# qurator-spk/sbb_textline_detection

Measured on AMD Instinct MI355X. Metric: segmented patches/sec (448x448x3) per GPU + per-pixel label-map match vs ref, higher is better.
Workload: dtype f16x3; 1 GPU; BASELINE configs[1] x 32: 32 pages of 3500x2500 (70 tiles of 448x448 each, margin 0.1) per GPU per step, textline model, 2 classes; workload_id=page, dedupe=False, max_batch=320, lanes=2, owned_regions=1, exchange=none

## Files before the change

sbb_textline_detection_amd/csrc/api.hip:

```cpp
#include <stdarg.h>
#include <stdio.h>
#include <stdlib.h>
#include <string.h>

#include <algorithm>
#include <cmath>
#include <new>
#include <stdexcept>
#include <string>
#include <utility>
#include <vector>

#include "../../include/sbbseg.h"
#include <dlfcn.h>

#include <mutex>

#include "internal.h"
#include "region.h"

using namespace sbbseg;

namespace {

// ... 208 lines not shown
    void* comm = nullptr;
    int comm_rank = 0, comm_world = 1;
    void* d_deskew = nullptr; size_t deskew_cap = 0;
    uint8_t *d_run_page = nullptr, *d_run_mask = nullptr, *d_run_a = nullptr, *d_run_b = nullptr;
    size_t run_page_cap = 0, run_mask_cap = 0, run_a_cap = 0, run_b_cap = 0;
    int *d_cc_parent = nullptr, *d_cc_count = nullptr; size_t cc_parent_cap = 0, cc_count_cap = 0;
    bool force_host_contours = false;
    int host_contour_calls = 0;
    int* d_cc_list = nullptr;
    int* d_cc_aux = nullptr; size_t cc_aux_cap = 0;
    unsigned long long* d_cc_small = nullptr;
    bool profiling = false;
    int conv_variant = 0;
    bool ph8 = false;
    int fg_min_ksteps = 9;
    int fg_pointwise_min_ksteps = 4;
    bool ranged_walk = false;
    bool block_pq = true;
    bool unfuse_blocks = false;
    bool unfuse_stem_pool = false;
    bool no_dec_halo = false;
    bool no_expand_reduce = false;
    bool no_c3er = false;
    bool plain_gather = false;
    int contig_max_k = 0;
    int fused_heads = 0;
    int num_cus = 256;
    std::vector<PendingEvent> pending;
    std::vector<hipEvent_t> free_events;
    int owned_mode = 1;
    int region_levels = 0;
    int region_op[kRegionMaxLevels] = {0};
    uint32_t* d_rtab[2][kRegionMaxLevels] = {{nullptr}, {nullptr}};
    size_t rtab_cap[2][kRegionMaxLevels] = {{0}, {0}};
    RegionRun rr;
    double last_exec_frac = 1.0;
    std::vector<std::pair<void*, size_t>> user_bufs;
};

namespace {

int dmalloc(sbbseg_ctx* c, void** p, size_t bytes)
{
    HIPCHK(hipMalloc(p, bytes));
    c->device_bytes += bytes;
    return 0;
// ... 193 lines not shown
                    HIPCHK(launch_stem_pool_x3(sp, c->num_cus, c->stream));
                } else
                    HIPCHK(launch_stem(sp, c->precision, c->num_cus, c->stream));
            } else if (co.d_d64_wfrag && !(c->conv_variant & 3)) {
                const Tensor& st = c->tensors[co.d.src[0].tensor];
                Direct64Params dp;
                dp.src = st.buf; dp.n = n; dp.H = st.H; dp.W = st.W; dp.wfrag = co.d_d64_wfrag;
                dp.scale = co.d_scale; dp.shift = co.d_shift; dp.relu = co.d.relu; dp.out = c->tensors[co.d.out_tensor].data();
                dp.wmul = co.wmul_cls[0];
                HIPCHK(launch_direct64(dp, c->precision, c->num_cus, c->stream));
            } else if (co.fused_reduce >= 0 && !c->no_expand_reduce && !(c->conv_variant & 3)) {
                const ConvOp& ro = c->ops[co.fused_reduce].conv;
                if (co.fused_conv3 >= 0 && !c->no_c3er) {
                    const ConvOp& k3 = c->ops[co.fused_conv3].conv;
                    const Tensor& ta = c->tensors[k3.d.src[0].tensor];
                    C3ERParams cp;
                    cp.a = ta.buf; cp.x = c->tensors[co.d.residual_tensor].buf;
                    cp.y = c->tensors[co.d.out_tensor].buf; cp.a2 = c->tensors[ro.d.out_tensor].buf;
                    cp.n = n; cp.H = ta.H; cp.W = ta.W; cp.C = co.d.src[0].channels; cp.x3 = c->precision == kF16X3;
                    cp.w2frag = co.d_c3_w2; cp.w3frag = co.d_er_w3; cp.w1frag = co.d_er_w1;
                    cp.s2 = k3.d_scale; cp.h2 = k3.d_shift; cp.s3 = co.d_scale; cp.h3 = co.d_shift; cp.s1 = ro.d_scale; cp.h1 = ro.d_shift;
                    cp.wmul2 = k3.wmul_cls[0]; cp.wmul3 = co.wmul_cls[0]; cp.wmul1 = ro.wmul_cls[0];
                    cp.k0 = co.d_c3_k0;
                    HIPCHK(launch_conv3_expand_reduce(cp, c->num_cus, c->stream));
                    return 0;
                }
                ExpRedParams ep;
                ep.b = c->tensors[co.d.src[0].tensor].buf; ep.x = c->tensors[co.d.residual_tensor].buf;
                ep.y = c->tensors[co.d.out_tensor].buf; ep.a2 = c->tensors[ro.d.out_tensor].buf;
                ep.M = n * co.Ho * co.Wo; ep.C = co.d.src[0].channels; ep.x3 = c->precision == kF16X3;
                ep.w3frag = co.d_er_w3; ep.w1frag = co.d_er_w1;
                ep.s3 = co.d_scale; ep.h3 = co.d_shift; ep.s1 = ro.d_scale; ep.h1 = ro.d_shift;
                ep.wmul3 = co.wmul_cls[0]; ep.wmul1 = ro.wmul_cls[0];
                ep.dbg = 0;
#ifdef SBBSEG_PROBES
                { static const int er_dbg = getenv("SBBSEG_ER_DBG") ? atoi(getenv("SBBSEG_ER_DBG")) : 0; ep.dbg = er_dbg; }
#endif
                HIPCHK(launch_expand_reduce_x3(ep, c->num_cus, c->stream));
            } else if (runs_dec_halo(c, co)) {
                const Tensor& s0 = c->tensors[co.d.src[0].tensor];
                DecHaloParams hp;
                hp.src0 = s0.buf; hp.skip = c->tensors[co.d.src[1].tensor].buf; hp.PH = s0.H; hp.PW = s0.W; hp.n = n;
                hp.wfrag = co.d_halo_wfrag; hp.taps = co.d_halo_taps; hp.scale = co.d_scale; hp.shift = co.d_shift;
                for (int q = 0; q < 4; ++q) hp.wmul[q] = co.wmul_cls[q];
                hp.relu = co.d.relu; hp.out = c->tensors[co.d.out_tensor].data();
                if (rlv >= 0) { hp.ttab = c->rr.tab[rlv]; hp.n_tab = c->rr.total[rlv]; }
                if (c->precision == kF16X3) HIPCHK(launch_dec_halo_x3(hp, c->num_cus, c->stream));
                else HIPCHK(launch_dec_halo_f16(hp, c->num_cus, c->stream));
            } else {
                int ks = 0;
                if (c->ksplit_now && n == 1 && c->precision != kF32 && p.fast_gather && conv_tile_bc(p.cout) == 128 && !p.raw_out && !p.head_classes &&
                    p.out && p.cout % 8 == 0 &&
                    ((p.n_cls == 1 && p.osy == 1 && p.osx == 1 && p.ooy == 0 && p.oox == 0 && p.TH == p.Ho && p.TW == p.Wo) ||
                     (p.n_cls == 4 && p.osy == 2 && p.osx == 2 && p.TH == 2 * p.Ho && p.TW == 2 * p.Wo))) {
                    const long tiles = (long)p.n_cls * ((p.M + 127) / 128) * ((p.cout + 127) / 128);
                    while (ks < 4 && (tiles << (ks + 1)) <= 512 && p.total_ksteps % (2 << ks) == 0 && (p.total_ksteps >> (ks + 1)) >= 4) ++ks;
                }
// ... 289 lines not shown
        const int words = (c->num_cus + 31) / 32, half = c->num_cus / 2;
        std::vector<uint32_t> lo(words, 0u), hi(words, 0u);
        for (int i = 0; i < c->num_cus; ++i) (i < half ? lo : hi)[i / 32] |= 1u << (i % 32);
        hipError_t e0 = hipExtStreamCreateWithCUMask(&c->half_stream[0], (uint32_t)words, lo.data());
        hipError_t e1 = e0 == hipSuccess ? hipExtStreamCreateWithCUMask(&c->half_stream[1], (uint32_t)words, hi.data()) : e0;
        if (e1 == hipSuccess) e1 = hipEventCreateWithFlags(&c->ev_half[0], hipEventDisableTiming);
        if (e1 == hipSuccess) e1 = hipEventCreateWithFlags(&c->ev_half[1], hipEventDisableTiming);
        if (e1 == hipSuccess) {
            c->cu_split = true;
            c->half_cus[0] = half; c->half_cus[1] = c->num_cus - half;
        } else {
            (void)hipGetLastError();
            for (int k = 0; k < 2; ++k) {
                if (c->half_stream[k]) (void)hipStreamDestroy(c->half_stream[k]);
                if (c->ev_half[k]) (void)hipEventDestroy(c->ev_half[k]);
                c->half_stream[k] = nullptr; c->ev_half[k] = nullptr;
            }
        }
    }
    if (const char* v = getenv("SBBSEG_STAGGER_MIN_TILES")) c->stagger_min_tiles = atoi(v);
    if (const char* v = getenv("SBBSEG_DEDUPE")) c->dedupe = v[0] != '0';
    if (const char* v = getenv("SBBSEG_KSPLIT")) c->ksplit = v[0] != '0';
    if (const char* v = getenv("SBBSEG_OWNED_REGIONS")) c->owned_mode = v[0] == '0' ? 0 : (v[0] == '2' ? 2 : 1);
    if (const char* v = getenv("SBBSEG_GRID_CUS")) { const int n = atoi(v); if (n >= 8 && n <= c->num_cus) c->num_cus = n & ~7; }
    *out = c;
    return 0;
    API_END
}

int sbbseg_destroy(sbbseg_ctx* c)
{
    API_BEGIN
    if (!c) return 0;
    (void)hipSetDevice(c->device);
    if (c->stream) (void)hipStreamSynchronize(c->stream);
    if (c->lane_stream) (void)hipStreamSynchronize(c->lane_stream);
    for (int k = 0; k < 2; ++k)
        if (c->half_stream[k]) (void)hipStreamSynchronize(c->half_stream[k]);
    for (auto& t : c->tensors) {
        (void)hipFree(t.lane_buf[0]);
        (void)hipFree(t.lane_buf[1]);
    }
    std::vector<Op*> all_ops;
    for (auto& op : c->ops) {
        all_ops.push_back(&op);
        for (auto& part : op.parts) all_ops.push_back(&part);
// ... 2535 lines not shown
```

sbb_textline_detection_amd/csrc/conv3_expand_reduce.hip:

```cpp
#include "internal.h"

namespace sbbseg {

namespace {

typedef __attribute__((ext_vector_type(8))) _Float16 h8_t;
typedef __attribute__((ext_vector_type(4))) _Float16 h4_t;
typedef __attribute__((ext_vector_type(2))) _Float16 h2_t;
typedef __attribute__((ext_vector_type(4))) float f4_t;
typedef __attribute__((ext_vector_type(4))) unsigned u4_t;
typedef __attribute__((ext_vector_type(2))) unsigned u2_t;
#define LDS_AS __attribute__((address_space(3)))

template <int N> struct IC { static constexpr int value = N; };
template <int B, int E, class F> __device__ __attribute__((always_inline)) inline void static_for(F&& f)
{
    if constexpr (B < E) {
        f(IC<B>{});
        static_for<B + 1, E>(f);
    }
}

__device__ inline f4_t mma(h8_t a, h8_t b, f4_t c) { return __builtin_amdgcn_mfma_f32_16x16x32_f16(a, b, c, 0, 0, 0); }

// ... 41 lines not shown
__device__ __attribute__((always_inline)) inline void glds16_hidden(const void* gsrc, uint32_t lds_dst)
{
    uint32_t keep;
    asm volatile("s_mov_b32 %0, m0\n\ts_mov_b32 m0, %2\n\ts_nop 0\n\tglobal_load_lds_dwordx4 %1, off\n\ts_mov_b32 m0, %0"
                 : "=&s"(keep) : "v"(gsrc), "s"(lds_dst) : "memory");
}
__device__ inline u4_t make_rsrc(const void* base, uint32_t bytes)
{
    u4_t r;
    const uint64_t b = (uint64_t)(uintptr_t)base;
    r[0] = __builtin_amdgcn_readfirstlane((uint32_t)b);
    r[1] = __builtin_amdgcn_readfirstlane((uint32_t)(b >> 32) & 0xffffu);
    r[2] = __builtin_amdgcn_readfirstlane(bytes);
    r[3] = 0x00020000u;
    return r;
}

constexpr int kHaloPx = 100;
constexpr int kHaloInstr = 25;
constexpr int kPieceBytes = kHaloInstr * 1024;

}

template <int C, bool X3>
__global__ __launch_bounds__(512, 2) void conv3_expand_reduce(const C3ERParams p)
{
    static_assert(C == 128, "stage 3 only (LDS: the split mode's halo + b + y chunk fill it at C = 128)");
    constexpr int EB = X3 ? 4 : 2;
    constexpr int KCH = X3 ? 32 : 64;
    constexpr int KS0 = 9 * C / KCH;
    constexpr int KS1 = C / KCH;
    constexpr int G2S = 256 / KCH;
    constexpr int NCH = C / 64;
    constexpr int MI2 = C / 128;
    constexpr int LG2 = 2 * MI2;
    constexpr int PB = C * EB, PY = 4 * C * EB, PA = C * EB;
    constexpr int NP = PB / 256;
    constexpr int YROW = 256 * EB;
    constexpr int SLB = PB / 16, SLY = YROW / 16;
    constexpr int kHaloBytes = NP * kPieceBytes, kBBytes = 64 * PB, kYBytes = 64 * YROW;
    constexpr int PER = KS1 + G2S;
    constexpr int STEPS = KS0 + NCH * PER;
    constexpr int kEpi1 = X3 ? 16 : 8, kEpi2 = X3 ? 8 : 4;
    constexpr int kDma = 4 * NP;
    static_assert(STEPS % 2 == 0 && KS0 % 2 == 0, "the weight ring alternates two register sets");
    extern __shared__ __attribute__((aligned(16))) char smem[];
    char* const lds_a = smem;
    char* const lds_b = smem + kHaloBytes;
    char* const lds_y = lds_b + kBBytes;
    float* const cst = (float*)(lds_y + kYBytes);
    const uint32_t lds0 = __builtin_amdgcn_readfirstlane((uint32_t)(uintptr_t)(LDS_AS char*)smem);

    const int tid = threadIdx.x;
    const int lane = tid & 63;
    const int wave = __builtin_amdgcn_readfirstlane(tid >> 6);
    const int frow = lane & 15, fg = lane >> 4;
    const int tiles_x = p.W >> 3, tiles_y = p.H >> 3;
    const int tpp = tiles_x * tiles_y;
    const int n_tiles = p.n * tpp;
    const int xcd = blockIdx.x & 7, slot = blockIdx.x >> 3, GX = gridDim.x >> 3;
    const int per_xcd = (n_tiles + 7) >> 3;
    const int xcd_lo = xcd * per_xcd, xcd_hi = min(n_tiles, xcd_lo + per_xcd);
    const int my_tiles = xcd_lo + slot < xcd_hi ? (xcd_hi - xcd_lo - slot + GX - 1) / GX : 0;
    if (my_tiles <= 0) return;
    auto tile_at = [&](int it) __attribute__((always_inline)) -> int { return xcd_lo + slot + (it < my_tiles ? it : my_tiles - 1) * GX; };
    auto tile_coords = [&](int tile, int& n, int& y0, int& x0) __attribute__((always_inline)) {
        n = tile / tpp;
// ... 86 lines not shown
#pragma unroll
        for (int ni = 0; ni < 4; ++ni) {
            dh[ni] = *(const h8_t*)(a + ni * 16 * row_bytes + (sh << 4));
            dl[ni] = *(const h8_t*)(a + ni * 16 * row_bytes + (sl << 4));
        }
    };
    auto load_halo = [&](int t, h8_t (&dh)[4], h8_t (&dl)[4]) __attribute__((always_inline)) {
        const int rec = k0[t];
        const int dy = (rec << 24) >> 24, dx = (rec << 16) >> 24, cg = rec >> 16;
        const int hp = a0 + dy * 10 + dx;
        const int sh = (r0 + 2 * dx + 8 * (cg & 1)) & 15;
        const char* base = lds_a + (cg >> 1) * kPieceBytes + hp * 256;
#pragma unroll
        for (int ni = 0; ni < 4; ++ni) {
            dh[ni] = *(const h8_t*)(base + ni * (20 * 256) + (sh << 4));
            dl[ni] = *(const h8_t*)(base + ni * (20 * 256) + (((sh + 4) & 15) << 4));
        }
    };

    int cn, cy0, cx0;
    tile_coords(tile_at(0), cn, cy0, cx0);
    uint32_t pix0 = (uint32_t)((cn * p.H + cy0) * p.W + cx0);
    issue_halo(tile_at(0));
    issue_x(pix0, 0);
    asm volatile("s_waitcnt vmcnt(0)" ::: "memory");
#pragma unroll
    for (int ni = 0; ni < 4; ++ni) {
        asm volatile("" : "+v"(xh[ni]));
        if constexpr (X3) asm volatile("" : "+v"(xl[ni]));
    }
    __syncthreads();
    issue_w(0, w[0]);
    issue_w(1, w[1]);

    for (int it = 0; it < my_tiles; ++it) {
        int nn, ny0, nx0;
        tile_coords(tile_at(it + 1), nn, ny0, nx0);
        const uint32_t pix_next = (uint32_t)((nn * p.H + ny0) * p.W + nx0);
        asm volatile("" : "+v"(rot), "+v"(xlane), "+v"(alane), "+v"(wlane), "+v"(frv), "+v"(fgv), "+v"(a0), "+v"(r0));
#pragma unroll
        for (int t = 0; t < KS0; ++t) asm volatile("" : "+s"(k0[t]));
        f4_t acc2[MI2][4];
        f4_t acc1[2][4];
        static_for<0, STEPS>([&](auto uc) __attribute__((always_inline)) {
            constexpr int u = decltype(uc)::value;
            constexpr bool g0 = u < KS0;
            constexpr int v = g0 ? 0 : u - KS0;
            constexpr int j = v / PER, r = v % PER;
            constexpr bool g1 = !g0 && r < KS1;
            constexpr int k = g0 ? u : (g1 ? r : r - KS1);
            constexpr int set = u & 1;
            constexpr int un = (u + 1) % STEPS;
            constexpr int Lnext = un < KS0 ? LG2 : (((un - KS0) % PER) < KS1 ? 4 : LG2);
            constexpr int extra = (!g0 && !g1 && k < 2) ? kEpi1 : ((g1 && j == 0 && k < 2) ? kDma : 0);
            if constexpr (g0 && k == 0) {
#pragma unroll
                for (int m = 0; m < MI2; ++m)
#pragma unroll
                    for (int ni = 0; ni < 4; ++ni) acc2[m][ni] = (f4_t){0.f, 0.f, 0.f, 0.f};
                load_halo(0, bh[set], bl[set]);
            }
            if constexpr (g1 && k == 0) {
#pragma unroll
                for (int m = 0; m < 2; ++m)
#pragma unroll
                    for (int ni = 0; ni < 4; ++ni) acc1[m][ni] = (f4_t){0.f, 0.f, 0.f, 0.f};
                load_frags(lds_b, PB, SLB, 0, bh[set], bl[set]);
            }
            if constexpr (!g0 && !g1 && k == 0) load_frags(lds_y, YROW, SLY, 0, bh[set], bl[set]);
            if constexpr (g0 && k + 1 < KS0) load_halo(k + 1, bh[set ^ 1], bl[set ^ 1]);
            if constexpr (g1 && k + 1 < KS1) load_frags(lds_b, PB, SLB, k + 1, bh[set ^ 1], bl[set ^ 1]);
            if constexpr (!g0 && !g1 && k + 1 < G2S) load_frags(lds_y, YROW, SLY, k + 1, bh[set ^ 1], bl[set ^ 1]);
            u4_t (&cw)[4] = w[set];
            if constexpr (g0 && k < 2) {
                wait4<Lnext>(cw[0], cw[1], cw[2], cw[3]);
            } else {
                wait4<Lnext + extra>(cw[0], cw[1], cw[2], cw[3]);
            }
            const h8_t (&ph)[4] = bh[set];
            const h8_t (&pl)[4] = bl[set];
            if constexpr (g1) {
                const h8_t ah[2] = {__builtin_bit_cast(h8_t, cw[0]), __builtin_bit_cast(h8_t, cw[2])};
                const h8_t al[2] = {__builtin_bit_cast(h8_t, cw[1]), __builtin_bit_cast(h8_t, cw[3])};
                if constexpr (X3) {
#pragma unroll
                    for (int m = 0; m < 2; ++m)
#pragma unroll
                        for (int ni = 0; ni < 4; ++ni) acc1[m][ni] = mma(al[m], ph[ni], acc1[m][ni]);
#pragma unroll
                    for (int m = 0; m < 2; ++m)
#pragma unroll
                        for (int ni = 0; ni < 4; ++ni) acc1[m][ni] = mma(ah[m], pl[ni], acc1[m][ni]);
                }
#pragma unroll
                for (int m = 0; m < 2; ++m)
// ... 61 lines not shown
                    } else if constexpr (X3) {
                        h4_t vh, vl;
                        split_n<4>(y, vh, vl);
                        *(h4_t*)(row + (s_hi << 4) + (boff & 8)) = vh;
                        *(h4_t*)(row + (s_lo << 4) + (boff & 8)) = vl;
                    } else if constexpr (MI2 == 2) {
                        u4_t vv;
                        vv[0] = pack_h2(y[0], y[1]); vv[1] = pack_h2(y[2], y[3]); vv[2] = pack_h2(y[4 % (4 * MI2)], y[5 % (4 * MI2)]); vv[3] = pack_h2(y[6 % (4 * MI2)], y[7 % (4 * MI2)]);
                        *(u4_t*)(row + (s_hi << 4)) = vv;
                    } else {
                        u2_t vv;
                        vv[0] = pack_h2(y[0], y[1]); vv[1] = pack_h2(y[2], y[3]);
                        *(u2_t*)(row + (s_hi << 4) + (boff & 8)) = vv;
                    }
                }
#pragma unroll
                for (int m = 0; m < MI2; ++m)
#pragma unroll
                    for (int ni = 0; ni < 4; ++ni) acc2[m][ni] = (f4_t){0.f, 0.f, 0.f, 0.f};
                asm volatile("s_waitcnt lgkmcnt(0)" ::: "memory");
                __builtin_amdgcn_s_barrier();
                asm volatile("" ::: "memory");
                issue_halo(tile_at(it + 1));
            }
            if constexpr (g1 && k == KS1 - 1) {
                if constexpr (X3)
                    asm volatile("s_waitcnt vmcnt(%8)" : "+v"(xh[0]), "+v"(xh[1]), "+v"(xh[2]), "+v"(xh[3]), "+v"(xl[0]), "+v"(xl[1]), "+v"(xl[2]), "+v"(xl[3])
                                 : "n"(2 * LG2) : "memory");
                else
                    asm volatile("s_waitcnt vmcnt(%4)" : "+v"(xh[0]), "+v"(xh[1]), "+v"(xh[2]), "+v"(xh[3]) : "n"(2 * LG2) : "memory");
                const int c0 = j * 256 + wave * 32 + fgv * 8;
                float sc[8], sh[8];
                *(float4*)&sc[0] = *(const float4*)(cst + c0); *(float4*)&sc[4] = *(const float4*)(cst + c0 + 4);
                *(float4*)&sh[0] = *(const float4*)(cst + 4 * C + c0); *(float4*)&sh[4] = *(const float4*)(cst + 4 * C + c0 + 4);
                const int s_hi = (wave * (X3 ? 8 : 4) + rot) & (SLY - 1), s_lo = (wave * 8 + 4 + rot) & (SLY - 1);
#pragma unroll
                for (int ni = 0; ni < 4; ++ni) {
                    float y[8];
#pragma unroll
                    for (int q = 0; q < 4; ++q) {
                        y[q] = __builtin_fmaf(acc1[0][ni][q], sc[q], sh[q]);
                        y[4 + q] = __builtin_fmaf(acc1[1][ni][q], sc[4 + q], sh[4 + q]);
                    }
                    const uint32_t off = xlane + pix0 * (uint32_t)PY + (uint32_t)ni * ni_y + (uint32_t)(j * YROW);
                    char* row = lds_y + (ni * 16 + frv) * YROW;
                    if constexpr (X3) {
                        const h8_t rh = __builtin_bit_cast(h8_t, xh[ni]), rl = __builtin_bit_cast(h8_t, xl[ni]);
#pragma unroll
                        for (int q = 0; q < 8; ++q) y[q] = fmaxf(__fadd_rn(y[q], __fadd_rn((float)rh[q], (float)rl[q])), 0.f);
                        h8_t vh, vl;
                        split_n<8>(y, vh, vl);
                        asm volatile("buffer_store_dwordx4 %1, %0, %3, 0 offen\n\tbuffer_store_dwordx4 %2, %0, %3, 0 offen offset:64\n\ts_nop 1"
                                     :: "v"(off), "v"(vh), "v"(vl), "s"(yrsrc) : "memory");
                        *(h8_t*)(row + (s_hi << 4)) = vh;
                        *(h8_t*)(row + (s_lo << 4)) = vl;
                    } else {
                        const h8_t rr = __builtin_bit_cast(h8_t, xh[ni]);
#pragma unroll
                        for (int q = 0; q < 8; ++q) y[q] = fmaxf(__fadd_rn(y[q], (float)rr[q]), 0.f);
                        u4_t vv;
                        vv[0] = pack_h2(y[0], y[1]); vv[1] = pack_h2(y[2], y[3]); vv[2] = pack_h2(y[4], y[5]); vv[3] = pack_h2(y[6], y[7]);
                        asm volatile("buffer_store_dwordx4 %1, %0, %2, 0 offen\n\ts_nop 1" :: "v"(off), "v"(vv), "s"(yrsrc) : "memory");
                        *(u4_t*)(row + (s_hi << 4)) = vv;
                    }
                }
                if constexpr (j + 1 < NCH) issue_x(pix0, j + 1);
                else issue_x(pix_next, 0);
                asm volatile("s_waitcnt lgkmcnt(0)" ::: "memory");
                __builtin_amdgcn_s_barrier();
                asm volatile("" ::: "memory");
            }
            if constexpr (!g0 && !g1 && k == G2S - 1) {
                asm volatile("s_waitcnt lgkmcnt(0)" ::: "memory");
                __builtin_amdgcn_s_barrier();
                asm volatile("" ::: "memory");
            }
        });

        {
            const int c0 = MI2 == 2 ? wave * 32 + fgv * 8 : (wave >> 1) * 32 + fgv * 8 + (wave & 1) * 4;
            float sc[4 * MI2], sh[4 * MI2];
            *(float4*)&sc[0] = *(const float4*)(cst + 8 * C + c0);
            *(float4*)&sh[0] = *(const float4*)(cst + 9 * C + c0);
            if constexpr (MI2 == 2) {
                *(float4*)&sc[4] = *(const float4*)(cst + 8 * C + c0 + 4);
                *(float4*)&sh[4] = *(const float4*)(cst + 9 * C + c0 + 4);
            }
#pragma unroll
            for (int ni = 0; ni < 4; ++ni) {
                const uint32_t off = alane + pix0 * (uint32_t)PA + (uint32_t)ni * ni_a;
// ... 5 lines not shown
                }
                if constexpr (X3 && MI2 == 2) {
                    h8_t vh, vl;
                    split_n<8>(y, vh, vl);
                    asm volatile("buffer_store_dwordx4 %1, %0, %3, 0 offen\n\tbuffer_store_dwordx4 %2, %0, %3, 0 offen offset:64\n\ts_nop 1"
                                 :: "v"(off), "v"(vh), "v"(vl), "s"(arsrc) : "memory");
                } else if constexpr (X3) {
                    h4_t vh, vl;
                    split_n<4>(y, vh, vl);
                    asm volatile("buffer_store_dwordx2 %1, %0, %3, 0 offen\n\tbuffer_store_dwordx2 %2, %0, %3, 0 offen offset:64\n\ts_nop 1"
                                 :: "v"(off), "v"(vh), "v"(vl), "s"(arsrc) : "memory");
                } else if constexpr (MI2 == 2) {
                    u4_t vv;
                    vv[0] = pack_h2(y[0], y[1]); vv[1] = pack_h2(y[2], y[3]); vv[2] = pack_h2(y[4 % (4 * MI2)], y[5 % (4 * MI2)]); vv[3] = pack_h2(y[6 % (4 * MI2)], y[7 % (4 * MI2)]);
                    asm volatile("buffer_store_dwordx4 %1, %0, %2, 0 offen\n\ts_nop 1" :: "v"(off), "v"(vv), "s"(arsrc) : "memory");
                } else {
                    u2_t vv;
                    vv[0] = pack_h2(y[0], y[1]); vv[1] = pack_h2(y[2], y[3]);
                    asm volatile("buffer_store_dwordx2 %1, %0, %2, 0 offen\n\ts_nop 1" :: "v"(off), "v"(vv), "s"(arsrc) : "memory");
                }
            }
        }
        pix0 = pix_next;
    }
    asm volatile("s_waitcnt vmcnt(0)" ::: "memory");
}

template <int C, bool X3> static hipError_t launch_one(const C3ERParams& p, int num_cus, hipStream_t s)
{
    constexpr int EB = X3 ? 4 : 2;
    constexpr int lds = (C * EB / 256) * kPieceBytes + 64 * C * EB + 64 * 256 * EB + 12 * C * 4;
    static_assert(lds <= 160 * 1024, "conv3_expand_reduce: LDS");
    static bool attr_done[64] = {};
    int dev = 0;
    hipError_t e = hipGetDevice(&dev);
    if (e != hipSuccess) return e;
    if (!attr_done[dev & 63]) {
        e = hipFuncSetAttribute((const void*)conv3_expand_reduce<C, X3>, hipFuncAttributeMaxDynamicSharedMemorySize, lds);
        if (e != hipSuccess) return e;
        attr_done[dev & 63] = true;
    }
    const int n_tiles = p.n * (p.H / 8) * (p.W / 8);
    if (n_tiles <= 0) return hipSuccess;
    const int grid = ((n_tiles < num_cus ? n_tiles : num_cus) + 7) & ~7;
    hipLaunchKernelGGL((conv3_expand_reduce<C, X3>), dim3(grid), dim3(512), lds, s, p);
    return hipGetLastError();
}

hipError_t launch_conv3_expand_reduce(const C3ERParams& p, int num_cus, hipStream_t s)
{
    if (p.C == 128) return p.x3 ? launch_one<128, true>(p, num_cus, s) : launch_one<128, false>(p, num_cus, s);
    return hipErrorInvalidValue;
}

}
```

sbb_textline_detection_amd/csrc/expand_reduce_x3.hip:

```cpp
#include "internal.h"

namespace sbbseg {

namespace {

typedef __attribute__((ext_vector_type(8))) _Float16 h8_t;
typedef __attribute__((ext_vector_type(4))) _Float16 h4_t;
typedef __attribute__((ext_vector_type(4))) float f4_t;
typedef __attribute__((ext_vector_type(4))) unsigned u4_t;
typedef __attribute__((ext_vector_type(2))) unsigned u2_t;
#define LDS_AS __attribute__((address_space(3)))

template <int N> struct IC { static constexpr int value = N; };
template <int B, int E, class F> __device__ __attribute__((always_inline)) inline void static_for(F&& f)
{
    if constexpr (B < E) {
        f(IC<B>{});
        static_for<B + 1, E>(f);
    }
}

__device__ inline f4_t mma(h8_t a, h8_t b, f4_t c) { return __builtin_amdgcn_mfma_f32_16x16x32_f16(a, b, c, 0, 0, 0); }

template <int N, class V> __device__ inline void split_n(const float (&y)[N], V& hi, V& lo)
// ... 39 lines not shown
template <int N> __device__ __attribute__((always_inline)) inline void wait4(u4_t& a, u4_t& b, u4_t& c, u4_t& d)
{
    asm volatile("s_waitcnt vmcnt(%4)" : "+v"(a), "+v"(b), "+v"(c), "+v"(d) : "n"(N) : "memory");
}
__device__ __attribute__((always_inline)) inline void glds16_hidden(const void* gsrc, uint32_t lds_dst)
{
    uint32_t keep;
    asm volatile("s_mov_b32 %0, m0\n\ts_mov_b32 m0, %2\n\ts_nop 0\n\tglobal_load_lds_dwordx4 %1, off\n\ts_mov_b32 m0, %0"
                 : "=&s"(keep) : "v"(gsrc), "s"(lds_dst) : "memory");
}
__device__ inline u4_t make_rsrc(const void* base, uint32_t bytes)
{
    u4_t r;
    const uint64_t b = (uint64_t)(uintptr_t)base;
    r[0] = __builtin_amdgcn_readfirstlane((uint32_t)b);
    r[1] = __builtin_amdgcn_readfirstlane((uint32_t)(b >> 32) & 0xffffu);
    r[2] = __builtin_amdgcn_readfirstlane(bytes);
    r[3] = 0x00020000u;
    return r;
}

}

template <int C, bool X3>
__global__ __launch_bounds__(512, 2) void expand_reduce(const ExpRedParams p)
{
    constexpr int EB = X3 ? 4 : 2;
    constexpr int KCH = X3 ? 32 : 64;
    constexpr int KS1 = C / KCH;
    constexpr int G2S = 256 / KCH;
    constexpr int NCH = C / 64;
    constexpr int MI2 = C / 128;
    constexpr int LG2 = 2 * MI2;
    constexpr int PB = C * EB, PY = 4 * C * EB, PA = C * EB;
    constexpr int YROW = 256 * EB;
    constexpr int SLB = PB / 16, SLY = YROW / 16;
    constexpr int kBBytes = 64 * PB, kYBytes = 64 * YROW;
    constexpr int STEPS = NCH * (KS1 + G2S);
    constexpr int kEpi1 = X3 ? 16 : 8, kEpi2 = X3 ? 8 : 4;
    extern __shared__ __attribute__((aligned(16))) char smem[];
    char* const lds_b = smem;
    char* const lds_y = smem + kBBytes;
    float* const cst = (float*)(smem + kBBytes + kYBytes);
    const uint32_t lds0 = __builtin_amdgcn_readfirstlane((uint32_t)(uintptr_t)(LDS_AS char*)smem);

    const int tid = threadIdx.x;
    const int lane = tid & 63;
    const int wave = __builtin_amdgcn_readfirstlane(tid >> 6);
    const int frow = lane & 15, fg = lane >> 4;
    const int n_tiles = (p.M + 63) >> 6;
    const int G = gridDim.x;
    const int my_tiles = (n_tiles - (int)blockIdx.x + G - 1) / G;
    if (my_tiles <= 0) return;
    auto tile_at = [&](int it) __attribute__((always_inline)) -> int { return (int)blockIdx.x + (it < my_tiles ? it : my_tiles - 1) * G; };

    for (int i = tid; i < 4 * C; i += 512) { cst[i] = p.s3[i] * p.wmul3; cst[4 * C + i] = p.h3[i]; }
    for (int i = tid; i < C; i += 512) { cst[8 * C + i] = p.s1[i] * p.wmul1; cst[9 * C + i] = p.h1[i]; }

    int dlane = lane;
    auto issue_b = [&](int tile) __attribute__((always_inline)) {
#pragma unroll
        for (int k = 0; k < KS1; ++k) {
// ... 28 lines not shown
        if (r < KS1) wload4(d[0], d[1], d[2], d[3], wlane + wm * (uint32_t)((j * KS1 + r) * 8 * 4096), w3rsrc);
        else if constexpr (MI2 == 2) wload4(d[0], d[1], d[2], d[3], wlane + wm * (uint32_t)((j * G2S + r - KS1) * 8 * 4096), w1rsrc);
        else wload2(d[0], d[1], wlane + wm * (uint32_t)((j * G2S + r - KS1) * 8 * 2048), w1rsrc);
    };
    auto issue_x = [&](int tile, int j) __attribute__((always_inline)) {
#pragma unroll
        for (int ni = 0; ni < 4; ++ni) {
            const uint32_t off = (SBBSEG_PROBE(p.dbg & 4) ? 0xf0000000u : 0u) + xlane + (uint32_t)(tile * 64 + ni * 16) * (uint32_t)PY + (uint32_t)(j * YROW);
            if constexpr (X3) xload2(xh[ni], xl[ni], off, xrsrc);
            else asm volatile("buffer_load_dwordx4 %0, %1, %2, 0 offen" : "=&v"(xh[ni]) : "v"(off), "s"(xrsrc) : "memory");
        }
    };
    auto load_frags = [&](const char* base, int row_bytes, int slots, int k, h8_t (&dh)[4], h8_t (&dl)[4]) __attribute__((always_inline)) {
        const int sh = (rot + 8 * k) & (slots - 1), sl = (rot + 8 * k + 4) & (slots - 1);
        const char* a = base + frv * row_bytes;
#pragma unroll
        for (int ni = 0; ni < 4; ++ni) {
            dh[ni] = *(const h8_t*)(a + ni * 16 * row_bytes + (sh << 4));
            dl[ni] = *(const h8_t*)(a + ni * 16 * row_bytes + (sl << 4));
        }
    };

    issue_b(tile_at(0));
    issue_x(tile_at(0), 0);
    asm volatile("s_waitcnt vmcnt(0)" ::: "memory");
#pragma unroll
    for (int ni = 0; ni < 4; ++ni) {
        asm volatile("" : "+v"(xh[ni]));
        if constexpr (X3) asm volatile("" : "+v"(xl[ni]));
    }
    __syncthreads();
    issue_w(0, w[0]);
    issue_w(1, w[1]);

    for (int it = 0; it < my_tiles; ++it) {
        const int tile = tile_at(it), tile_next = tile_at(it + 1);
        asm volatile("" : "+v"(rot), "+v"(xlane), "+v"(alane), "+v"(wlane), "+v"(dlane), "+v"(frv), "+v"(fgv));
        f4_t acc2[MI2][4];
#pragma unroll
        for (int m = 0; m < MI2; ++m)
#pragma unroll
            for (int ni = 0; ni < 4; ++ni) acc2[m][ni] = (f4_t){0.f, 0.f, 0.f, 0.f};
        f4_t acc1[2][4];
        static_for<0, STEPS>([&](auto uc) __attribute__((always_inline)) {
            constexpr int u = decltype(uc)::value;
            constexpr int j = u / (KS1 + G2S), r = u % (KS1 + G2S);
            constexpr bool g1 = r < KS1;
            constexpr int k = g1 ? r : r - KS1;
            constexpr int set = u & 1;
            constexpr int un = (u + 1) % STEPS;
            constexpr int Lnext = (un % (KS1 + G2S)) < KS1 ? 4 : LG2;
            constexpr int extra = (!g1 && k < 2) ? kEpi1 + (j == NCH - 1 ? KS1 : 0) : 0;
            if constexpr (g1 && k == 0) {
#pragma unroll
                for (int m = 0; m < 2; ++m)
#pragma unroll
                    for (int ni = 0; ni < 4; ++ni) acc1[m][ni] = (f4_t){0.f, 0.f, 0.f, 0.f};
                load_frags(lds_b, PB, SLB, 0, bh[set], bl[set]);
            }
            if constexpr (!g1 && k == 0) load_frags(lds_y, YROW, SLY, 0, bh[set], bl[set]);
            if constexpr (g1 && k + 1 < KS1) load_frags(lds_b, PB, SLB, k + 1, bh[set ^ 1], bl[set ^ 1]);
            if constexpr (!g1 && k + 1 < G2S) load_frags(lds_y, YROW, SLY, k + 1, bh[set ^ 1], bl[set ^ 1]);
            u4_t (&cw)[4] = w[set];
            if constexpr (g1 && j == 0 && k < 2) {
                wait4<Lnext>(cw[0], cw[1], cw[2], cw[3]);
            } else {
                wait4<Lnext + extra>(cw[0], cw[1], cw[2], cw[3]);
            }
            const h8_t (&ph)[4] = bh[set];
            const h8_t (&pl)[4] = bl[set];
            if constexpr (g1) {
                const h8_t ah[2] = {__builtin_bit_cast(h8_t, cw[0]), __builtin_bit_cast(h8_t, cw[2])};
                const h8_t al[2] = {__builtin_bit_cast(h8_t, cw[1]), __builtin_bit_cast(h8_t, cw[3])};
                if constexpr (X3) {
#pragma unroll
                    for (int m = 0; m < 2; ++m)
#pragma unroll
                        for (int ni = 0; ni < 4; ++ni) acc1[m][ni] = mma(al[m], ph[ni], acc1[m][ni]);
#pragma unroll
                    for (int m = 0; m < 2; ++m)
#pragma unroll
                        for (int ni = 0; ni < 4; ++ni) acc1[m][ni] = mma(ah[m], pl[ni], acc1[m][ni]);
                }
#pragma unroll
                for (int m = 0; m < 2; ++m)
#pragma unroll
                    for (int ni = 0; ni < 4; ++ni) acc1[m][ni] = mma(ah[m], ph[ni], acc1[m][ni]);
                if constexpr (!X3) {
// ... 10 lines not shown
#pragma unroll
                    for (int m = 0; m < MI2; ++m)
#pragma unroll
                        for (int ni = 0; ni < 4; ++ni) acc2[m][ni] = mma(al[m], ph[ni], acc2[m][ni]);
#pragma unroll
                    for (int m = 0; m < MI2; ++m)
#pragma unroll
                        for (int ni = 0; ni < 4; ++ni) acc2[m][ni] = mma(ah[m], pl[ni], acc2[m][ni]);
                }
#pragma unroll
                for (int m = 0; m < MI2; ++m)
#pragma unroll
                    for (int ni = 0; ni < 4; ++ni) acc2[m][ni] = mma(ah[m], ph[ni], acc2[m][ni]);
                if constexpr (!X3) {
#pragma unroll
                    for (int m = 0; m < MI2; ++m)
#pragma unroll
                        for (int ni = 0; ni < 4; ++ni) acc2[m][ni] = mma(al[m], pl[ni], acc2[m][ni]);
                }
            }
            issue_w((u + 2) % STEPS, cw);
            __builtin_amdgcn_sched_barrier(0);

            if constexpr (g1 && k == KS1 - 1) {
                if constexpr (X3)
                    asm volatile("s_waitcnt vmcnt(%8)" : "+v"(xh[0]), "+v"(xh[1]), "+v"(xh[2]), "+v"(xh[3]), "+v"(xl[0]), "+v"(xl[1]), "+v"(xl[2]), "+v"(xl[3])
                                 : "n"(2 * LG2) : "memory");
                else
                    asm volatile("s_waitcnt vmcnt(%4)" : "+v"(xh[0]), "+v"(xh[1]), "+v"(xh[2]), "+v"(xh[3]) : "n"(2 * LG2) : "memory");
                const int c0 = j * 256 + wave * 32 + fgv * 8;
                float sc[8], sh[8];
                *(float4*)&sc[0] = *(const float4*)(cst + c0); *(float4*)&sc[4] = *(const float4*)(cst + c0 + 4);
                *(float4*)&sh[0] = *(const float4*)(cst + 4 * C + c0); *(float4*)&sh[4] = *(const float4*)(cst + 4 * C + c0 + 4);
                const int s_hi = (wave * (X3 ? 8 : 4) + rot) & (SLY - 1), s_lo = (wave * 8 + 4 + rot) & (SLY - 1);
#pragma unroll
                for (int ni = 0; ni < 4; ++ni) {
                    float y[8];
#pragma unroll
                    for (int q = 0; q < 4; ++q) {
                        y[q] = __builtin_fmaf(acc1[0][ni][q], sc[q], sh[q]);
                        y[4 + q] = __builtin_fmaf(acc1[1][ni][q], sc[4 + q], sh[4 + q]);
                    }
                    const uint32_t off = (SBBSEG_PROBE(p.dbg & 2) ? 0xf0000000u : 0u) + xlane + (uint32_t)(tile * 64 + ni * 16) * (uint32_t)PY + (uint32_t)(j * YROW);
                    char* row = lds_y + (ni * 16 + frv) * YROW;
                    if constexpr (X3) {
                        const h8_t rh = __builtin_bit_cast(h8_t, xh[ni]), rl = __builtin_bit_cast(h8_t, xl[ni]);
#pragma unroll
                        for (int q = 0; q < 8; ++q) y[q] = fmaxf(__fadd_rn(y[q], __fadd_rn((float)rh[q], (float)rl[q])), 0.f);
                        h8_t vh, vl;
                        split_n<8>(y, vh, vl);
                        asm volatile("buffer_store_dwordx4 %1, %0, %3, 0 offen\n\tbuffer_store_dwordx4 %2, %0, %3, 0 offen offset:64\n\ts_nop 1"
                                     :: "v"(off), "v"(vh), "v"(vl), "s"(yrsrc) : "memory");
                        *(h8_t*)(row + (s_hi << 4)) = vh;
                        *(h8_t*)(row + (s_lo << 4)) = vl;
                    } else {
                        const h8_t rr = __builtin_bit_cast(h8_t, xh[ni]);
#pragma unroll
                        for (int q = 0; q < 8; ++q) y[q] = fmaxf(__fadd_rn(y[q], (float)rr[q]), 0.f);
                        u4_t v;
                        v[0] = pack_h2(y[0], y[1]); v[1] = pack_h2(y[2], y[3]); v[2] = pack_h2(y[4], y[5]); v[3] = pack_h2(y[6], y[7]);
                        asm volatile("buffer_store_dwordx4 %1, %0, %2, 0 offen\n\ts_nop 1" :: "v"(off), "v"(v), "s"(yrsrc) : "memory");
                        *(u4_t*)(row + (s_hi << 4)) = v;
                    }
                }
                if constexpr (j + 1 < NCH) issue_x(tile, j + 1);
                else issue_x(tile_next, 0);
                asm volatile("s_waitcnt lgkmcnt(0)" ::: "memory");
                __builtin_amdgcn_s_barrier();
                asm volatile("" ::: "memory");
                if constexpr (j == NCH - 1) issue_b(tile_next);
            }
            if constexpr (!g1 && k == G2S - 1) {
                asm volatile("s_waitcnt lgkmcnt(0)" ::: "memory");
                __builtin_amdgcn_s_barrier();
                asm volatile("" ::: "memory");
            }
        });

        {
            const int c0 = MI2 == 2 ? wave * 32 + fgv * 8 : (wave >> 1) * 32 + fgv * 8 + (wave & 1) * 4;
            float sc[4 * MI2], sh[4 * MI2];
            *(float4*)&sc[0] = *(const float4*)(cst + 8 * C + c0);
            *(float4*)&sh[0] = *(const float4*)(cst + 9 * C + c0);
            if constexpr (MI2 == 2) {
                *(float4*)&sc[4] = *(const float4*)(cst + 8 * C + c0 + 4);
                *(float4*)&sh[4] = *(const float4*)(cst + 9 * C + c0 + 4);
            }
#pragma unroll
            for (int ni = 0; ni < 4; ++ni) {
                const uint32_t off = alane + (uint32_t)(tile * 64 + ni * 16) * (uint32_t)PA;
                float y[4 * MI2];
#pragma unroll
                for (int q = 0; q < 4; ++q) {
// ... 2 lines not shown
                }
                if constexpr (X3 && MI2 == 2) {
                    h8_t vh, vl;
                    split_n<8>(y, vh, vl);
                    asm volatile("buffer_store_dwordx4 %1, %0, %3, 0 offen\n\tbuffer_store_dwordx4 %2, %0, %3, 0 offen offset:64\n\ts_nop 1"
                                 :: "v"(off), "v"(vh), "v"(vl), "s"(arsrc) : "memory");
                } else if constexpr (X3) {
                    h4_t vh, vl;
                    split_n<4>(y, vh, vl);
                    asm volatile("buffer_store_dwordx2 %1, %0, %3, 0 offen\n\tbuffer_store_dwordx2 %2, %0, %3, 0 offen offset:64\n\ts_nop 1"
                                 :: "v"(off), "v"(vh), "v"(vl), "s"(arsrc) : "memory");
                } else if constexpr (MI2 == 2) {
                    u4_t v;
                    v[0] = pack_h2(y[0], y[1]); v[1] = pack_h2(y[2], y[3]); v[2] = pack_h2(y[4 % (4 * MI2)], y[5 % (4 * MI2)]); v[3] = pack_h2(y[6 % (4 * MI2)], y[7 % (4 * MI2)]);
                    asm volatile("buffer_store_dwordx4 %1, %0, %2, 0 offen\n\ts_nop 1" :: "v"(off), "v"(v), "s"(arsrc) : "memory");
                } else {
                    u2_t v;
                    v[0] = pack_h2(y[0], y[1]); v[1] = pack_h2(y[2], y[3]);
                    asm volatile("buffer_store_dwordx2 %1, %0, %2, 0 offen\n\ts_nop 1" :: "v"(off), "v"(v), "s"(arsrc) : "memory");
                }
            }
        }
    }
    asm volatile("s_waitcnt vmcnt(0)" ::: "memory");
}

template <int C, bool X3> static hipError_t launch_one(const ExpRedParams& p, int num_cus, hipStream_t s)
{
    constexpr int EB = X3 ? 4 : 2;
    constexpr int lds = 64 * C * EB + 64 * 256 * EB + 10 * C * 4;
    static bool attr_done[64] = {};
    int dev = 0;
    hipError_t e = hipGetDevice(&dev);
    if (e != hipSuccess) return e;
    if (!attr_done[dev & 63]) {
        e = hipFuncSetAttribute((const void*)expand_reduce<C, X3>, hipFuncAttributeMaxDynamicSharedMemorySize, lds);
        if (e != hipSuccess) return e;
        attr_done[dev & 63] = true;
    }
    const int n_tiles = (p.M + 63) / 64;
    const int grid = n_tiles < num_cus ? n_tiles : num_cus;
    hipLaunchKernelGGL((expand_reduce<C, X3>), dim3(grid), dim3(512), lds, s, p);
    return hipGetLastError();
}

hipError_t launch_expand_reduce_x3(const ExpRedParams& p, int num_cus, hipStream_t s)
{
    if (p.C == 128) return p.x3 ? launch_one<128, true>(p, num_cus, s) : launch_one<128, false>(p, num_cus, s);
    if (p.C == 256) return p.x3 ? launch_one<256, true>(p, num_cus, s) : launch_one<256, false>(p, num_cus, s);
    return hipErrorInvalidValue;
}

}
```

sbb_textline_detection_amd/csrc/internal.h:

```cpp
#pragma once
#include <hip/hip_runtime.h>
#include <stdint.h>

namespace sbbseg {

constexpr int kZeroHeaderBytes = 256;
constexpr int kBK = 64;
constexpr int kGranulesPerStep = 8;

struct SrcDesc {
    const char* base;
    int PH, PW;
    int pix_bytes;
    int shift;
    int lim_y, lim_x;
    int ksteps;
    int sy_shift, sx_shift;
    int lo_off;
    uint32_t bytes;
    int tap_lo_y, tap_lo_x;
};

struct KTabEntry {
    int16_t dy, dx;
// ... 148 lines not shown
    const float* scale;
    const float* shift;
    float wmul[4];
    int relu;
    void* out;
    const uint32_t* ttab = nullptr;
    int n_tab = 0;
};

struct ExpRedParams {
    const char* b;
    const char* x;
    char* y;
    char* a2;
    int M;
    int C;
    int x3;
    const void* w3frag;
    const void* w1frag;
    const float *s3, *h3;
    const float *s1, *h1;
    float wmul3, wmul1;
    int dbg;
};

struct C3ERParams {
    const char* a;
    const char* x;
    char* y;
    char* a2;
    int n, H, W;
    int C;
    int x3;
    const void* w2frag;
    const void* w3frag;
    const void* w1frag;
    const float *s2, *h2;
    const float *s3, *h3;
    const float *s1, *h1;
    float wmul2, wmul3, wmul1;
    const int* k0;
};

struct HeadParams {
    const void* src;
    int cin;
    int classes;
    int M;
    const float* w;
    const float* scale;
    const float* shift;
    uint8_t* labels;
    float* probs;
};

struct IngestParams {
    const uint8_t* page;
    int Hp, Wp;
    int src_Hp, src_Wp;
    int whole;
    const int* tile_xy;
    int grid_first, grid_nyf;
    int grid_mid_x, grid_mid_y;
    int n_tiles;
// ... 65 lines not shown
```

Baseline: 5821 patches/s.

## Phase-stagger wave groups in expand-reduce kernels to overlap GEMM halves

Adds a phased schedule to the fused expand-reduce and conv3-expand-reduce kernels, enabled by default. The two wave groups are offset by one barrier so that half of each GEMM runs in one group while the other group is in the other half. The residual x loads are moved to the start of each expand chunk, and extra mid-GEMM barriers are inserted. The aim is to spread LDS and epilogue contention across the waves and overlap the two phases. The cost is more barriers and more complex vmcnt bookkeeping, which could cause stalls or ordering bugs.

```diff
diff --git a/sbb_textline_detection_amd/csrc/api.hip b/sbb_textline_detection_amd/csrc/api.hip
--- a/sbb_textline_detection_amd/csrc/api.hip
+++ b/sbb_textline_detection_amd/csrc/api.hip
@@ -254,6 +254,7 @@
     bool no_dec_halo = false;
     bool no_expand_reduce = false;
     bool no_c3er = false;
+    bool er_phased = true;
     bool plain_gather = false;
     int contig_max_k = 0;
     int fused_heads = 0;
@@ -493,6 +494,7 @@
                     cp.s2 = k3.d_scale; cp.h2 = k3.d_shift; cp.s3 = co.d_scale; cp.h3 = co.d_shift; cp.s1 = ro.d_scale; cp.h1 = ro.d_shift;
                     cp.wmul2 = k3.wmul_cls[0]; cp.wmul3 = co.wmul_cls[0]; cp.wmul1 = ro.wmul_cls[0];
                     cp.k0 = co.d_c3_k0;
+                    cp.phased = c->er_phased;
                     HIPCHK(launch_conv3_expand_reduce(cp, c->num_cus, c->stream));
                     return 0;
                 }
@@ -504,6 +506,7 @@
                 ep.s3 = co.d_scale; ep.h3 = co.d_shift; ep.s1 = ro.d_scale; ep.h1 = ro.d_shift;
                 ep.wmul3 = co.wmul_cls[0]; ep.wmul1 = ro.wmul_cls[0];
                 ep.dbg = 0;
+                ep.phased = c->er_phased;
 #ifdef SBBSEG_PROBES
                 { static const int er_dbg = getenv("SBBSEG_ER_DBG") ? atoi(getenv("SBBSEG_ER_DBG")) : 0; ep.dbg = er_dbg; }
 #endif
@@ -839,6 +842,7 @@
     if (const char* v = getenv("SBBSEG_DEDUPE")) c->dedupe = v[0] != '0';
     if (const char* v = getenv("SBBSEG_KSPLIT")) c->ksplit = v[0] != '0';
     if (const char* v = getenv("SBBSEG_OWNED_REGIONS")) c->owned_mode = v[0] == '0' ? 0 : (v[0] == '2' ? 2 : 1);
+    if (const char* v = getenv("SBBSEG_ER_PHASED")) c->er_phased = v[0] != '0';
     if (const char* v = getenv("SBBSEG_GRID_CUS")) { const int n = atoi(v); if (n >= 8 && n <= c->num_cus) c->num_cus = n & ~7; }
     *out = c;
     return 0;
diff --git a/sbb_textline_detection_amd/csrc/conv3_expand_reduce.hip b/sbb_textline_detection_amd/csrc/conv3_expand_reduce.hip
--- a/sbb_textline_detection_amd/csrc/conv3_expand_reduce.hip
+++ b/sbb_textline_detection_amd/csrc/conv3_expand_reduce.hip
@@ -87,7 +87,7 @@
 
 }
 
-template <int C, bool X3>
+template <int C, bool X3, bool PH>
 __global__ __launch_bounds__(512, 2) void conv3_expand_reduce(const C3ERParams p)
 {
     static_assert(C == 128, "stage 3 only (LDS: the split mode's halo + b + y chunk fill it at C = 128)");
@@ -108,6 +108,9 @@
     constexpr int STEPS = KS0 + NCH * PER;
     constexpr int kEpi1 = X3 ? 16 : 8, kEpi2 = X3 ? 8 : 4;
     constexpr int kDma = 4 * NP;
+    constexpr int H1 = KS1 / 2, H2 = G2S / 2;
+    constexpr int kX = X3 ? 8 : 4, kY = kEpi1 - kX;
+    static_assert(KS1 % 2 == 0 && G2S % 2 == 0, "the phased schedule halves both GEMMs");
     static_assert(STEPS % 2 == 0 && KS0 % 2 == 0, "the weight ring alternates two register sets");
     extern __shared__ __attribute__((aligned(16))) char smem[];
     char* const lds_a = smem;
@@ -240,7 +243,7 @@
     tile_coords(tile_at(0), cn, cy0, cx0);
     uint32_t pix0 = (uint32_t)((cn * p.H + cy0) * p.W + cx0);
     issue_halo(tile_at(0));
-    issue_x(pix0, 0);
+    if constexpr (!PH) issue_x(pix0, 0);
     asm volatile("s_waitcnt vmcnt(0)" ::: "memory");
 #pragma unroll
     for (int ni = 0; ni < 4; ++ni) {
@@ -250,6 +253,7 @@
     __syncthreads();
     issue_w(0, w[0]);
     issue_w(1, w[1]);
+    const bool group_b = wave >= 4;
 
     for (int it = 0; it < my_tiles; ++it) {
         int nn, ny0, nx0;
@@ -270,7 +274,8 @@
             constexpr int set = u & 1;
             constexpr int un = (u + 1) % STEPS;
             constexpr int Lnext = un < KS0 ? LG2 : (((un - KS0) % PER) < KS1 ? 4 : LG2);
-            constexpr int extra = (!g0 && !g1 && k < 2) ? kEpi1 : ((g1 && j == 0 && k < 2) ? kDma : 0);
+            constexpr int extra = (!g0 && !g1 && k < 2) ? (PH ? kY : kEpi1) : (g1 && k < 2 ? (j == 0 ? kDma : 0) + (PH ? kX : 0) : 0);
+            if constexpr (PH && g1 && k == 0) issue_x(pix0, j);
             if constexpr (g0 && k == 0) {
 #pragma unroll
                 for (int m = 0; m < MI2; ++m)
@@ -285,10 +290,10 @@
                     for (int ni = 0; ni < 4; ++ni) acc1[m][ni] = (f4_t){0.f, 0.f, 0.f, 0.f};
                 load_frags(lds_b, PB, SLB, 0, bh[set], bl[set]);
             }
-            if constexpr (!g0 && !g1 && k == 0) load_frags(lds_y, YROW, SLY, 0, bh[set], bl[set]);
+            if constexpr (!g0 && !g1 && (k == 0 || (PH && k == H2))) load_frags(lds_y, YROW, SLY, k, bh[set], bl[set]);
             if constexpr (g0 && k + 1 < KS0) load_halo(k + 1, bh[set ^ 1], bl[set ^ 1]);
             if constexpr (g1 && k + 1 < KS1) load_frags(lds_b, PB, SLB, k + 1, bh[set ^ 1], bl[set ^ 1]);
-            if constexpr (!g0 && !g1 && k + 1 < G2S) load_frags(lds_y, YROW, SLY, k + 1, bh[set ^ 1], bl[set ^ 1]);
+            if constexpr (!g0 && !g1 && k + 1 < G2S && !(PH && k + 1 == H2)) load_frags(lds_y, YROW, SLY, k + 1, bh[set ^ 1], bl[set ^ 1]);
             u4_t (&cw)[4] = w[set];
             if constexpr (g0 && k < 2) {
                 wait4<Lnext>(cw[0], cw[1], cw[2], cw[3]);
@@ -396,6 +401,19 @@
                 __builtin_amdgcn_s_barrier();
                 asm volatile("" ::: "memory");
                 issue_halo(tile_at(it + 1));
+                if constexpr (PH) {
+                    if (group_b) __builtin_amdgcn_s_barrier();
+                    asm volatile("" ::: "memory");
+                }
+            }
+            if constexpr (PH && g1 && k == H1 - 1) {
+                __builtin_amdgcn_s_barrier();
+                asm volatile("" ::: "memory");
+            }
+            if constexpr (PH && g1 && k == KS1 - 1) {
+                asm volatile("s_waitcnt lgkmcnt(0)" ::: "memory");
+                __builtin_amdgcn_s_barrier();
+                asm volatile("" ::: "memory");
             }
             if constexpr (g1 && k == KS1 - 1) {
                 if constexpr (X3)
@@ -438,8 +456,15 @@
                         *(u4_t*)(row + (s_hi << 4)) = vv;
                     }
                 }
-                if constexpr (j + 1 < NCH) issue_x(pix0, j + 1);
-                else issue_x(pix_next, 0);
+                if constexpr (!PH) {
+                    if constexpr (j + 1 < NCH) issue_x(pix0, j + 1);
+                    else issue_x(pix_next, 0);
+                }
+                asm volatile("s_waitcnt lgkmcnt(0)" ::: "memory");
+                __builtin_amdgcn_s_barrier();
+                asm volatile("" ::: "memory");
+            }
+            if constexpr (PH && !g0 && !g1 && k == H2 - 1) {
                 asm volatile("s_waitcnt lgkmcnt(0)" ::: "memory");
                 __builtin_amdgcn_s_barrier();
                 asm volatile("" ::: "memory");
@@ -491,11 +516,15 @@
             }
         }
         pix0 = pix_next;
+        if constexpr (PH) {
+            if (!group_b) __builtin_amdgcn_s_barrier();
+            asm volatile("" ::: "memory");
+        }
     }
     asm volatile("s_waitcnt vmcnt(0)" ::: "memory");
 }
 
-template <int C, bool X3> static hipError_t launch_one(const C3ERParams& p, int num_cus, hipStream_t s)
+template <int C, bool X3, bool PH> static hipError_t launch_one(const C3ERParams& p, int num_cus, hipStream_t s)
 {
     constexpr int EB = X3 ? 4 : 2;
     constexpr int lds = (C * EB / 256) * kPieceBytes + 64 * C * EB + 64 * 256 * EB + 12 * C * 4;
@@ -505,20 +534,21 @@
     hipError_t e = hipGetDevice(&dev);
     if (e != hipSuccess) return e;
     if (!attr_done[dev & 63]) {
-        e = hipFuncSetAttribute((const void*)conv3_expand_reduce<C, X3>, hipFuncAttributeMaxDynamicSharedMemorySize, lds);
+        e = hipFuncSetAttribute((const void*)conv3_expand_reduce<C, X3, PH>, hipFuncAttributeMaxDynamicSharedMemorySize, lds);
         if (e != hipSuccess) return e;
         attr_done[dev & 63] = true;
     }
     const int n_tiles = p.n * (p.H / 8) * (p.W / 8);
     if (n_tiles <= 0) return hipSuccess;
     const int grid = ((n_tiles < num_cus ? n_tiles : num_cus) + 7) & ~7;
-    hipLaunchKernelGGL((conv3_expand_reduce<C, X3>), dim3(grid), dim3(512), lds, s, p);
+    hipLaunchKernelGGL((conv3_expand_reduce<C, X3, PH>), dim3(grid), dim3(512), lds, s, p);
     return hipGetLastError();
 }
 
 hipError_t launch_conv3_expand_reduce(const C3ERParams& p, int num_cus, hipStream_t s)
 {
-    if (p.C == 128) return p.x3 ? launch_one<128, true>(p, num_cus, s) : launch_one<128, false>(p, num_cus, s);
+    if (p.C == 128 && p.phased) return p.x3 ? launch_one<128, true, true>(p, num_cus, s) : launch_one<128, false, true>(p, num_cus, s);
+    if (p.C == 128) return p.x3 ? launch_one<128, true, false>(p, num_cus, s) : launch_one<128, false, false>(p, num_cus, s);
     return hipErrorInvalidValue;
 }
 
diff --git a/sbb_textline_detection_amd/csrc/expand_reduce_x3.hip b/sbb_textline_detection_amd/csrc/expand_reduce_x3.hip
--- a/sbb_textline_detection_amd/csrc/expand_reduce_x3.hip
+++ b/sbb_textline_detection_amd/csrc/expand_reduce_x3.hip
@@ -85,7 +85,7 @@
 
 }
 
-template <int C, bool X3>
+template <int C, bool X3, bool PH>
 __global__ __launch_bounds__(512, 2) void expand_reduce(const ExpRedParams p)
 {
     constexpr int EB = X3 ? 4 : 2;
@@ -101,6 +101,9 @@
     constexpr int kBBytes = 64 * PB, kYBytes = 64 * YROW;
     constexpr int STEPS = NCH * (KS1 + G2S);
     constexpr int kEpi1 = X3 ? 16 : 8, kEpi2 = X3 ? 8 : 4;
+    constexpr int H1 = KS1 / 2, H2 = G2S / 2;
+    constexpr int kX = X3 ? 8 : 4, kY = kEpi1 - kX;
+    static_assert(KS1 % 2 == 0 && G2S % 2 == 0 && H2 >= 2, "the phased schedule halves both GEMMs");
     extern __shared__ __attribute__((aligned(16))) char smem[];
     char* const lds_b = smem;
     char* const lds_y = smem + kBBytes;
@@ -175,7 +178,7 @@
     };
 
     issue_b(tile_at(0));
-    issue_x(tile_at(0), 0);
+    if constexpr (!PH) issue_x(tile_at(0), 0);
     asm volatile("s_waitcnt vmcnt(0)" ::: "memory");
 #pragma unroll
     for (int ni = 0; ni < 4; ++ni) {
@@ -185,6 +188,8 @@
     __syncthreads();
     issue_w(0, w[0]);
     issue_w(1, w[1]);
+    const bool group_b = wave >= 4;
+    if (PH && group_b) __builtin_amdgcn_s_barrier();
 
     for (int it = 0; it < my_tiles; ++it) {
         const int tile = tile_at(it), tile_next = tile_at(it + 1);
@@ -203,7 +208,9 @@
             constexpr int set = u & 1;
             constexpr int un = (u + 1) % STEPS;
             constexpr int Lnext = (un % (KS1 + G2S)) < KS1 ? 4 : LG2;
-            constexpr int extra = (!g1 && k < 2) ? kEpi1 + (j == NCH - 1 ? KS1 : 0) : 0;
+            constexpr int extra = PH ? ((!g1 && k < 2) ? kY + (j == NCH - 1 ? KS1 : 0) : ((g1 && k < 2) ? kX : 0))
+                                     : ((!g1 && k < 2) ? kEpi1 + (j == NCH - 1 ? KS1 : 0) : 0);
+            if constexpr (PH && g1 && k == 0) issue_x(tile, j);
             if constexpr (g1 && k == 0) {
 #pragma unroll
                 for (int m = 0; m < 2; ++m)
@@ -211,12 +218,12 @@
                     for (int ni = 0; ni < 4; ++ni) acc1[m][ni] = (f4_t){0.f, 0.f, 0.f, 0.f};
                 load_frags(lds_b, PB, SLB, 0, bh[set], bl[set]);
             }
-            if constexpr (!g1 && k == 0) load_frags(lds_y, YROW, SLY, 0, bh[set], bl[set]);
+            if constexpr (!g1 && (k == 0 || (PH && k == H2))) load_frags(lds_y, YROW, SLY, k, bh[set], bl[set]);
             if constexpr (g1 && k + 1 < KS1) load_frags(lds_b, PB, SLB, k + 1, bh[set ^ 1], bl[set ^ 1]);
-            if constexpr (!g1 && k + 1 < G2S) load_frags(lds_y, YROW, SLY, k + 1, bh[set ^ 1], bl[set ^ 1]);
+            if constexpr (!g1 && k + 1 < G2S && !(PH && k + 1 == H2)) load_frags(lds_y, YROW, SLY, k + 1, bh[set ^ 1], bl[set ^ 1]);
             u4_t (&cw)[4] = w[set];
             if constexpr (g1 && j == 0 && k < 2) {
-                wait4<Lnext>(cw[0], cw[1], cw[2], cw[3]);
+                wait4<Lnext + (PH ? kX : 0)>(cw[0], cw[1], cw[2], cw[3]);
             } else {
                 wait4<Lnext + extra>(cw[0], cw[1], cw[2], cw[3]);
             }
@@ -273,6 +280,15 @@
             issue_w((u + 2) % STEPS, cw);
             __builtin_amdgcn_sched_barrier(0);
 
+            if constexpr (PH && g1 && k == H1 - 1) {
+                __builtin_amdgcn_s_barrier();
+                asm volatile("" ::: "memory");
+            }
+            if constexpr (PH && g1 && k == KS1 - 1) {
+                asm volatile("s_waitcnt lgkmcnt(0)" ::: "memory");
+                __builtin_amdgcn_s_barrier();
+                asm volatile("" ::: "memory");
+            }
             if constexpr (g1 && k == KS1 - 1) {
                 if constexpr (X3)
                     asm volatile("s_waitcnt vmcnt(%8)" : "+v"(xh[0]), "+v"(xh[1]), "+v"(xh[2]), "+v"(xh[3]), "+v"(xl[0]), "+v"(xl[1]), "+v"(xl[2]), "+v"(xl[3])
@@ -314,12 +330,20 @@
                         *(u4_t*)(row + (s_hi << 4)) = v;
                     }
                 }
-                if constexpr (j + 1 < NCH) issue_x(tile, j + 1);
-                else issue_x(tile_next, 0);
+                if constexpr (!PH) {
+                    if constexpr (j + 1 < NCH) issue_x(tile, j + 1);
+                    else issue_x(tile_next, 0);
+                }
                 asm volatile("s_waitcnt lgkmcnt(0)" ::: "memory");
                 __builtin_amdgcn_s_barrier();
                 asm volatile("" ::: "memory");
                 if constexpr (j == NCH - 1) issue_b(tile_next);
+            }
+            if constexpr (PH && !g1 && k == H2 - 1) {
+                if constexpr (j == NCH - 1 && H2 <= 2) asm volatile("s_waitcnt vmcnt(%0)" :: "n"(H2 * LG2) : "memory");
+                asm volatile("s_waitcnt lgkmcnt(0)" ::: "memory");
+                __builtin_amdgcn_s_barrier();
+                asm volatile("" ::: "memory");
             }
             if constexpr (!g1 && k == G2S - 1) {
                 asm volatile("s_waitcnt lgkmcnt(0)" ::: "memory");
@@ -368,10 +392,11 @@
             }
         }
     }
+    if (PH && !group_b) __builtin_amdgcn_s_barrier();
     asm volatile("s_waitcnt vmcnt(0)" ::: "memory");
 }
 
-template <int C, bool X3> static hipError_t launch_one(const ExpRedParams& p, int num_cus, hipStream_t s)
+template <int C, bool X3, bool PH> static hipError_t launch_one(const ExpRedParams& p, int num_cus, hipStream_t s)
 {
     constexpr int EB = X3 ? 4 : 2;
     constexpr int lds = 64 * C * EB + 64 * 256 * EB + 10 * C * 4;
@@ -380,20 +405,25 @@
     hipError_t e = hipGetDevice(&dev);
     if (e != hipSuccess) return e;
     if (!attr_done[dev & 63]) {
-        e = hipFuncSetAttribute((const void*)expand_reduce<C, X3>, hipFuncAttributeMaxDynamicSharedMemorySize, lds);
+        e = hipFuncSetAttribute((const void*)expand_reduce<C, X3, PH>, hipFuncAttributeMaxDynamicSharedMemorySize, lds);
         if (e != hipSuccess) return e;
         attr_done[dev & 63] = true;
     }
     const int n_tiles = (p.M + 63) / 64;
     const int grid = n_tiles < num_cus ? n_tiles : num_cus;
-    hipLaunchKernelGGL((expand_reduce<C, X3>), dim3(grid), dim3(512), lds, s, p);
+    hipLaunchKernelGGL((expand_reduce<C, X3, PH>), dim3(grid), dim3(512), lds, s, p);
     return hipGetLastError();
 }
 
+template <int C, bool X3> static hipError_t launch_sched(const ExpRedParams& p, int num_cus, hipStream_t s)
+{
+    return p.phased ? launch_one<C, X3, true>(p, num_cus, s) : launch_one<C, X3, false>(p, num_cus, s);
+}
+
 hipError_t launch_expand_reduce_x3(const ExpRedParams& p, int num_cus, hipStream_t s)
 {
-    if (p.C == 128) return p.x3 ? launch_one<128, true>(p, num_cus, s) : launch_one<128, false>(p, num_cus, s);
-    if (p.C == 256) return p.x3 ? launch_one<256, true>(p, num_cus, s) : launch_one<256, false>(p, num_cus, s);
+    if (p.C == 128) return p.x3 ? launch_sched<128, true>(p, num_cus, s) : launch_sched<128, false>(p, num_cus, s);
+    if (p.C == 256) return p.x3 ? launch_sched<256, true>(p, num_cus, s) : launch_sched<256, false>(p, num_cus, s);
     return hipErrorInvalidValue;
 }
 
diff --git a/sbb_textline_detection_amd/csrc/internal.h b/sbb_textline_detection_amd/csrc/internal.h
--- a/sbb_textline_detection_amd/csrc/internal.h
+++ b/sbb_textline_detection_amd/csrc/internal.h
@@ -194,6 +194,7 @@
     const float *s1, *h1;
     float wmul3, wmul1;
     int dbg;
+    int phased = 1;
 };
 
 struct C3ERParams {
@@ -212,6 +213,7 @@
     const float *s1, *h1;
     float wmul2, wmul3, wmul1;
     const int* k0;
+    int phased = 1;
 };
 
 struct HeadParams {
```

New measurement: 5811 patches/s, median of 2. Within noise of the previous version (-0.2%).
